# eceo-epfl/ScaleProtoSeg

Hardware: AMD Instinct MI355X
Metric: Mpix/s fwd+bwd prototype-distance, Cityscapes 1024x2048 (higher is better)
Workload: dtype bf16; 1 GPU; cityscapes_1024x2048_c256_p190_s1; latent_px_per_gpu=2097152, channels=256, prototypes=190, scales=1, classes=19, features_dtype=bf16, parallelism=single

## Files before the change

### scaleprotoseg_amd/csrc/spx_bank.hip

```cpp
#include "spx_args.h"
#include "spx_common.h"
#include <type_traits>

#define SPX_BK_THREADS 512
#define SPX_BANK_PIPE 1
#define SPX_BANK_STAGGER 1
__host__ __device__ constexpr int spx_bk_row(int cpx) { return 2 * cpx + 16; }

__host__ __device__ inline int spx_bk_wstride(const spx_plan& pl) {
    return ((pl.channels_per_scale + 31) / 32) * 32 + pl.ncb * 32 + 32;
}
static void spx_bank_parts(const spx_plan& pl, int B, int HW, int& nci, int& nci_vec, int& slabs_vec, int& slabs_tail) {
    nci = 2 * ((HW + SPX_TILE_PX - 1) / SPX_TILE_PX);
    nci_vec = HW >= 8 ? nci : 0;
    long long cap = 256 / pl.npanels;
    if (cap < 1) cap = 1;
    const long long cv = (long long)B * nci_vec, ct = (long long)B * (nci - nci_vec);
    slabs_vec = (int)(cv < cap ? cv : cap);
    slabs_tail = (int)(ct < cap ? ct : cap);
}
int spx_bank_bwd_nsplit(const spx_plan& pl, int B, int HW) {
    int nci, nci_vec, sv, st;
    spx_bank_parts(pl, B, HW, nci, nci_vec, sv, st);
    return sv + st;
}
size_t spx_bank_bwd_ws_floats(const spx_plan& pl, int nsplit) {
    return (size_t)nsplit * pl.npanels * pl.npb * 32 * spx_bk_wstride(pl);
}
template <int NPB, int NCB, bool DO_P, bool DO_W, int CPX>
__host__ __device__ constexpr int spx_bk_buf_bytes() {
    constexpr int fb = (CPX / 32) * NPB * 2 * 1024;
    return (DO_P ? fb + 256 * spx_bk_row(CPX) : 0) + (DO_W ? 2 * fb + 2 * NCB * 32 * spx_bk_row(CPX) : 0);
}
template <int NPB, int NCB, bool DO_P, bool DO_W, int CPX>
__host__ __device__ constexpr int spx_bk_lds_bytes() {
    constexpr int red = (2 * 3 * 2 * 1024 + 2 * 3 * 64) * 4;
    constexpr int n = (CPX == 32 ? 2 : 1) * spx_bk_buf_bytes<NPB, NCB, DO_P, DO_W, CPX>();
    return (n > red ? n : red) + 16;
}

template <int NPB, int NCB, bool XF32, int VM, bool DO_P, bool DO_W, bool KSPLIT, int CPX>
__global__ __launch_bounds__(SPX_BK_THREADS, 2) void spx_bank_bwd_kernel(const SpxBankBwdArgs a) {
    constexpr bool VEC = VM != 0, RAG = VM == 2;
    constexpr int SPX_BK_PX = CPX, SPX_BK_ROW = spx_bk_row(CPX);
    constexpr int NW1 = CPX / 32;
    constexpr bool PIPE = CPX == 32;
    static_assert(!(PIPE && KSPLIT), "the k-step split needs four pixel k-steps per chunk");
    extern __shared__ __attribute__((aligned(16))) char smem[];
    const spx_plan& pl = a.plan;
    const int tid = threadIdx.x, lane = tid & 63;
    const int wave = __builtin_amdgcn_readfirstlane(tid >> 6);
    const int r = lane & 31, h = lane >> 5;
    const int q = blockIdx.y, split = blockIdx.x;
    const int Cs = pl.channels_per_scale, K = pl.num_classes;
    const int C = pl.num_scales * Cs;
    const int nchb = (Cs + 31) / 32;
    constexpr int rows = NPB * 32;
    const int ch0 = pl.panel_ch0[q];
    const int tiles_per_img = (a.HW + SPX_TILE_PX - 1) / SPX_TILE_PX;
    const size_t ntiles = (size_t)a.B * tiles_per_img;
    static_assert(CPX == 64 || CPX == 32, "chunk width");
    const int nci = a.nci_launch * (64 / CPX);
    const int ci0 = a.ci_first * (64 / CPX);
    const long long total = (long long)a.B * nci;
    const long long cstep = a.nslabs;
    int phase = split;
    if (CPX == 32 && (a.nslabs & 15) == 0) {
        const int xcd = split & 7, slot = split >> 3;
        phase = 2 * ((slot >> 1) * 8 + xcd) + (slot & 1);
    }
    const long long c_begin = phase;
    const long long c_end = total;
    const bool want_w = DO_W && a.d_W != nullptr;
    const bool want_p = DO_P && a.d_bank != nullptr;
    constexpr int ESZ = XF32 ? 4 : 2;
    constexpr int NFRAG = NW1 * NPB * 2;
    constexpr int FBYTES = NFRAG * 1024;

    constexpr int BUF = spx_bk_buf_bytes<NPB, NCB, DO_P, DO_W, CPX>();
    int32_t* const ebuf = (int32_t*)(smem + spx_bk_lds_bytes<NPB, NCB, DO_P, DO_W, CPX>() - 16);
    char *Gs, *Xs, *As, *As2, *Ls, *Ls2;
    int cur_buf = 0;
    auto use_buffer = [&](int buf) {
        cur_buf = buf;
        Gs = smem + buf * BUF;
        Xs = Gs + (DO_P ? FBYTES : 0);
        As = Xs + (DO_P ? 256 * SPX_BK_ROW : 0);
        As2 = As + FBYTES;
        Ls = As2 + FBYTES;
        Ls2 = Ls + NCB * 32 * SPX_BK_ROW;
    };
    use_buffer(0);

    const int cpair = wave & 3;
    constexpr int PH = NPB / 2;
    const int pb0 = (wave >> 2) * PH;
    const bool w_role = wave < NPB;
    constexpr bool ksplit = KSPLIT;
    const int cs_first = wave >> 2;
    auto cs_owner = [&](int i) { return i == 0 ? cs_first : i + 1; };

    f32x16 accp[PH][2];
    f32x16 accw[NCB];
    float csum[PH];
    int e_acc = 0;
    bool have_e = false;
#pragma unroll
    for (int i = 0; i < PH; ++i) {
        csum[i] = 0.0f;
#pragma unroll
        for (int t = 0; t < 2; ++t)
#pragma unroll
            for (int e = 0; e < 16; ++e) accp[i][t][e] = 0.0f;
    }
#pragma unroll
    for (int cb = 0; cb < NCB; ++cb)
#pragma unroll
        for (int e = 0; e < 16; ++e) accw[cb][e] = 0.0f;

    constexpr int FP = (FBYTES / 16 + SPX_BK_THREADS - 1) / SPX_BK_THREADS;
    constexpr int PPR = CPX / 8;
    constexpr int RPP = SPX_BK_THREADS / PPR;
    constexpr int XPT = 256 / RPP;
    struct Stage {
        u32x4 gr[FP], ar[FP], xr[XPT][XF32 ? 2 : 1];
        uint32_t exw[FP];
        float lr_[(CPX * 32 * NCB + SPX_BK_THREADS - 1) / SPX_BK_THREADS];
        int32_t gexp;
        uint32_t rot_bits;
        bool ragged;
    };
    Stage stg[PIPE ? 2 : 1];
    uint32_t gsc_off[FP];
#pragma unroll
    for (int i = 0; i < FP; ++i) {
        const int off = (i * SPX_BK_THREADS + tid) * 16;
        const int frag = off >> 10, slot = (off >> 4) & 63, s2 = frag & 1;
        const int t = (slot - 8 * s2) & 63;
        const int rr = (t >> 3) * 4 + (t & 3), hh = (t & 7) >> 2;
        gsc_off[i] = off < FBYTES ? (uint32_t)(((frag >> 1) * 64 + rr + 32 * hh) * 4) : SPX_OOB;
    }
    const size_t blob_total = (size_t)pl.npanels * ntiles * 4 * NPB * 2 * 1024;
    constexpr int LPT = (SPX_BK_PX * 32 * NCB + SPX_BK_THREADS - 1) / SPX_BK_THREADS;
    const int piece = tid % PPR, prow = tid / PPR;

    long long nx_c = c_begin;
    int nx_b = (int)(c_begin / nci);
    int nx_ci = (int)(c_begin - (long long)nx_b * nci);
    const int step_b = (int)(cstep / nci), step_ci = (int)(cstep - (long long)step_b * nci);
    auto issue = [&](Stage& st) {
        const int b = nx_b;
        const int ci = ci0 + nx_ci;
        if (nx_c + cstep < c_end) {
            nx_c += cstep;
            nx_b += step_b;
            nx_ci += step_ci;
            if (nx_ci >= nci) {
                nx_ci -= nci;
                ++nx_b;
            }
        }
        constexpr int CPT = SPX_TILE_PX / CPX;
        const size_t tile_g = (size_t)b * tiles_per_img + ci / CPT;
        const size_t blob0 = ((((size_t)q * ntiles + tile_g) * 4 + NW1 * (ci % CPT)) * NPB * 2) * 1024;
        const spx_rsrc grs = make_rsrc_pred(a.g_in ? (const char*)a.g_in + blob0 : nullptr);
        const spx_rsrc ars = make_rsrc_pred(a.a_in ? (const char*)a.a_in + blob0 : nullptr);
        const char* const exsrc = (want_w && a.a_in) ? (const char*)a.a_in : nullptr;
        const spx_rsrc exs = make_rsrc_pred(exsrc ? exsrc + blob_total + blob0 / 8 : nullptr);
        st.gexp = (want_p && a.g_in) ? *(const int32_t*)((const char*)a.g_in + spx_gexp_offset(blob_total) + ((size_t)q * ntiles + tile_g) * 4) : 0;
#pragma unroll
        for (int i = 0; i < FP; ++i) {
            const uint32_t off = (uint32_t)((i * SPX_BK_THREADS + tid) * 16);
            st.gr[i] = buf_load_b128(grs, (want_p && off < (uint32_t)FBYTES) ? off : SPX_OOB, 0);
            st.exw[i] = (uint32_t)__builtin_amdgcn_raw_buffer_load_b32(exs, exsrc ? gsc_off[i] : SPX_OOB, 0, 0);
            st.ar[i] = buf_load_b128(ars, (want_w && off < (uint32_t)FBYTES) ? off : SPX_OOB, 0);
        }
        const int px = ci * SPX_BK_PX + piece * 8;
        {
            const int over = px + 8 - a.HW;
            st.rot_bits = (RAG && over > 0 && over < 8) ? (uint32_t)over * (ESZ * 8) : 0u;
            st.ragged = RAG && (ci * SPX_BK_PX + SPX_BK_PX > a.HW);
        }
#pragma unroll
        for (int i = 0; i < XPT; ++i) {
            const int row = prow + RPP * i;
            const spx_rsrc xb = make_rsrc_pred((const char*)a.x + ((size_t)b * C + ch0 + RPP * i) * a.HW * ESZ);
            const uint32_t vo = ((uint32_t)prow * (uint32_t)a.HW + (uint32_t)px) * ESZ;
            const bool row_ok = want_p && row < Cs;
            if (VEC) {
                const int over = px + 8 - a.HW;
                const uint32_t v = !row_ok ? SPX_OOB : (over <= 0 ? vo : ((RAG && over < 8) ? vo - (uint32_t)over * ESZ : SPX_OOB));
                st.xr[i][0] = buf_load_b128(xb, v, 0);
                if (XF32) st.xr[i][1] = buf_load_b128(xb, v == SPX_OOB ? SPX_OOB : v + 16, 0);
            } else if (XF32) {
#pragma unroll
                for (int e = 0; e < 8; ++e)
                    st.xr[i][e >> 2][e & 3] = __float_as_uint(buf_load_f32(xb, (row_ok && px + e < a.HW) ? vo + 4 * e : SPX_OOB, 0));
            } else {
#pragma unroll
                for (int e = 0; e < 4; ++e) {
                    const uint32_t lo = buf_load_u16(xb, (row_ok && px + 2 * e < a.HW) ? vo + 4 * e : SPX_OOB, 0);
                    const uint32_t hi = buf_load_u16(xb, (row_ok && px + 2 * e + 1 < a.HW) ? vo + 4 * e + 2 : SPX_OOB, 0);
                    st.xr[i][0][e] = lo | (hi << 16);
                }
            }
        }
        const int px0 = ci * SPX_BK_PX;
        const spx_rsrc lb = make_rsrc_pred(a.d_logits ? a.d_logits + ((size_t)b * a.HW + px0) * K : nullptr);
#pragma unroll
        for (int i = 0; i < LPT; ++i) {
            const int e = i * SPX_BK_THREADS + tid;
            const int p = e / K;
            st.lr_[i] = buf_load_f32(lb, (want_w && e < SPX_BK_PX * K && px0 + p < a.HW) ? (uint32_t)e * 4u : SPX_OOB, 0);
        }
    };

    auto commit = [&](Stage& st) {
#pragma unroll
        for (int i = 0; i < FP; ++i) {
            const int off = (i * SPX_BK_THREADS + tid) * 16;
            if (off < FBYTES) {
                if (DO_P) *(u32x4*)(Gs + off) = st.gr[i];
                if (DO_W) {
                    u32x4 ahw, alw;
                    const float asc = __builtin_amdgcn_ldexpf(1.0f / SPX_ABLOB_I16_ONE, (int)((st.exw[i] >> 8) & 0xffu) - 128);
#pragma unroll
                    for (int j = 0; j < 4; ++j) {
                        f32x2 v;
                        v[0] = (float)(short)(st.ar[i][j] & 0xffffu);
                        v[1] = (float)((int)st.ar[i][j] >> 16);
                        uint32_t hi, lo;
                        split_bf16x2(v * asc, hi, lo);
                        ahw[j] = hi;
                        alw[j] = lo;
                    }
                    *(u32x4*)(As + off) = ahw;
                    *(u32x4*)(As2 + off) = alw;
                }
            }
        }
        if (DO_P && tid == 0) ebuf[cur_buf] = st.gexp;
        if (RAG && st.ragged) {
#pragma unroll
            for (int i = 0; i < XPT; ++i) {
                if (XF32) spx_shr256(st.xr[i][0], st.xr[i][XF32 ? 1 : 0], st.rot_bits);
                else st.xr[i][0] = spx_shr128(st.xr[i][0], st.rot_bits);
            }
        }
#pragma unroll
        for (int i = 0; i < XPT; ++i) {
            u32x4 v;
            if (XF32) {
#pragma unroll
                for (int e = 0; e < 4; ++e) {
                    f32x2 p;
                    p[0] = (float)(__bf16)__uint_as_float(st.xr[i][e >> 1][(2 * e) & 3]);
                    p[1] = (float)(__bf16)__uint_as_float(st.xr[i][e >> 1][(2 * e + 1) & 3]);
                    v[e] = pack_f16x2_rtz(p);
                }
            } else {
#pragma unroll
                for (int e = 0; e < 4; ++e) v[e] = pack_f16x2_rtz(unpack_bf16x2(st.xr[i][0][e]));
            }
            if (DO_P) *(u32x4*)(Xs + (prow + RPP * i) * SPX_BK_ROW + piece * 16) = v;
        }
#pragma unroll
        for (int i = 0; i < LPT; ++i) {
            const int e = i * SPX_BK_THREADS + tid;
            if (DO_W && e < SPX_BK_PX * K) {
                const int p = e / K, cls = e - p * K;
                __bf16 hi, lo;
                split_bf16(st.lr_[i], hi, lo);
                *(uint16_t*)(Ls + cls * SPX_BK_ROW + p * 2) = __builtin_bit_cast(uint16_t, hi);
                *(uint16_t*)(Ls2 + cls * SPX_BK_ROW + p * 2) = __builtin_bit_cast(uint16_t, lo);
            }
        }
    };

    for (int buf = 0; buf < (PIPE ? 2 : 1); ++buf) {
        use_buffer(buf);
        for (int e = tid; DO_W && e < NCB * 32 * SPX_BK_PX; e += SPX_BK_THREADS) {
            const int cls = e / SPX_BK_PX, p = e - cls * SPX_BK_PX;
            if (cls >= K) {
                *(uint16_t*)(Ls + cls * SPX_BK_ROW + p * 2) = 0;
                *(uint16_t*)(Ls2 + cls * SPX_BK_ROW + p * 2) = 0;
            }
        }
    }
    use_buffer(0);

    const int tg = lane >> 4, tli = lane & 15, tqq = tli >> 2, tpp = tli & 3;
    const int ts2 = tg & 1, tkh = tg >> 1;

    auto chunk_scale = [&]() -> bool {
        const int e_c = __builtin_amdgcn_readfirstlane(ebuf[cur_buf]);
        if (have_e && e_c == e_acc) return true;
        if (have_e && e_c - e_acc > 80) return false;
        const float ratio = have_e ? __builtin_amdgcn_ldexpf(1.0f, e_c - e_acc) : 1.0f;
#pragma unroll
        for (int i = 0; i < PH; ++i) {
            csum[i] *= ratio;
#pragma unroll
            for (int t = 0; t < 2; ++t)
#pragma unroll
                for (int e = 0; e < 16; ++e) accp[i][t][e] *= ratio;
        }
        e_acc = e_c;
        have_e = true;
        return true;
    };
    auto bank_part = [&](int ks, int cp) {
        const int koff = (ks * 16 + 8 * h) * 2;
        const int pxa = ks * 16 + 8 * tkh + tqq;
        const int wsel = pxa >> 5, ra = pxa & 31;
        const int fo0 = spx_blob_slot(ra, tpp & 1, ts2) * 16 + 8 * (tpp >> 1);
        const int fo1 = spx_blob_slot(ra + 4, tpp & 1, ts2) * 16 + 8 * (tpp >> 1);
        f16x8 xb[2];
#pragma unroll
        for (int t = 0; t < 2; ++t) xb[t] = *(const f16x8*)(Xs + ((2 * cp + t) * 32 + r) * SPX_BK_ROW + koff);
#pragma unroll
        for (int i = 0; i < PH; ++i) {
            const int fb = ((wsel * NPB + pb0 + i) * 2 + ts2) * 1024;
            const s16x4 g0 = lds_tr_read(Gs + fb + fo0);
            const s16x4 g1 = lds_tr_read(Gs + fb + fo1);
            const f16x8 gf = __builtin_bit_cast(f16x8, __builtin_shufflevector(g0, g1, 0, 1, 2, 3, 4, 5, 6, 7));
            if (ksplit || cpair == cs_owner(i)) {
                f16x2 one2;
                one2[0] = (_Float16)1.0f;
                one2[1] = (_Float16)1.0f;
                float s8 = csum[i];
#pragma unroll
                for (int e = 0; e < 4; ++e) {
                    f16x2 pr;
                    pr[0] = gf[2 * e];
                    pr[1] = gf[2 * e + 1];
                    s8 = __builtin_amdgcn_fdot2(pr, one2, s8, false);
                }
                csum[i] = s8;
            }
#pragma unroll
            for (int t = 0; t < 2; ++t) accp[i][t] = __builtin_amdgcn_mfma_f32_32x32x16_f16(gf, xb[t], accp[i][t], 0, 0, 0);
        }
    };
    auto head_part = [&](int ks) {
        const int koff = (ks * 16 + 8 * h) * 2;
        const int pxa = ks * 16 + 8 * tkh + tqq;
        const int wsel = pxa >> 5, ra = pxa & 31;
        const int fo0 = spx_blob_slot(ra, tpp & 1, ts2) * 16 + 8 * (tpp >> 1);
        const int fo1 = spx_blob_slot(ra + 4, tpp & 1, ts2) * 16 + 8 * (tpp >> 1);
        const int fb = ((wsel * NPB + wave) * 2 + ts2) * 1024;
        const bf16x4 a0 = __builtin_bit_cast(bf16x4, lds_tr_read(As + fb + fo0));
        const bf16x4 a1 = __builtin_bit_cast(bf16x4, lds_tr_read(As + fb + fo1));
        const bf16x4 b0 = __builtin_bit_cast(bf16x4, lds_tr_read(As2 + fb + fo0));
        const bf16x4 b1 = __builtin_bit_cast(bf16x4, lds_tr_read(As2 + fb + fo1));
        const bf16x8 af = __builtin_shufflevector(a0, a1, 0, 1, 2, 3, 4, 5, 6, 7);
        const bf16x8 af2 = __builtin_shufflevector(b0, b1, 0, 1, 2, 3, 4, 5, 6, 7);
#pragma unroll
        for (int cb = 0; cb < NCB; ++cb) {
            const bf16x8 lf = *(const bf16x8*)(Ls + (cb * 32 + r) * SPX_BK_ROW + koff);
            const bf16x8 lf2 = *(const bf16x8*)(Ls2 + (cb * 32 + r) * SPX_BK_ROW + koff);
            accw[cb] = mfma_bf16(af, lf, accw[cb]);
            accw[cb] = mfma_bf16(af2, lf, accw[cb]);
            accw[cb] = mfma_bf16(af, lf2, accw[cb]);
        }
    };
    auto compute = [&]() {
        const bool add_p = DO_P && chunk_scale();
        if constexpr (KSPLIT) {
            if (add_p) bank_part(cpair, 0);
            if (DO_W && w_role) {
#pragma unroll
                for (int ks = 0; ks < SPX_BK_PX / 16; ++ks) head_part(ks);
            }
        } else {
#pragma unroll
            for (int ks = 0; ks < SPX_BK_PX / 16; ++ks) {
                if (add_p) bank_part(ks, cpair);
                if (DO_W && w_role) head_part(ks);
            }
        }
    };
    if constexpr (!PIPE) {
        if (c_begin < c_end) issue(stg[0]);
        for (long long c = c_begin; c < c_end; c += cstep) {
            commit(stg[0]);
            __syncthreads();
            issue(stg[0]);
            __builtin_amdgcn_sched_barrier(0);
            compute();
            __syncthreads();
        }
    } else if (c_begin < c_end) {
        const bool late = SPX_BANK_STAGGER && wave >= 4;
        const int la = late ? 1 : 0;
        issue(stg[0]);
        commit(stg[0]);
        if (!late) {
            issue(stg[0]);
            issue(stg[1]);
        } else {
            issue(stg[1]);
            issue(stg[0]);
            use_buffer(1);
            commit(stg[1]);
            issue(stg[1]);
        }
        __syncthreads();
        for (long long c = c_begin; c < c_end; c += 2 * cstep) {
            use_buffer(0);
            compute();
            if (late) __syncthreads();
            use_buffer(1 - la);
            commit(stg[0]);
            issue(stg[0]);
            if (!late) __syncthreads();
            if (c + cstep < c_end) {
                use_buffer(1);
                compute();
                if (late) __syncthreads();
                use_buffer(la);
                commit(stg[1]);
                issue(stg[1]);
                if (!late) __syncthreads();
            }
        }
    }

    if (DO_P && ksplit && want_p) {
        float* const red = (float*)smem;
        float* const redc = red + 2 * 3 * 2 * 1024;
        const int half = wave >> 2;
#pragma unroll
        for (int i = 0; i < PH; ++i) {
            __syncthreads();
            if (cpair > 0) {
#pragma unroll
                for (int t = 0; t < 2; ++t)
#pragma unroll
                    for (int reg = 0; reg < 16; ++reg)
                        red[(((half * 3 + cpair - 1) * 2 + t) * 16 + reg) * 64 + lane] = accp[i][t][reg];
                redc[(half * 3 + cpair - 1) * 64 + lane] = csum[i];
            }
            __syncthreads();
            if (cpair == 0) {
#pragma unroll
                for (int c = 0; c < 3; ++c) {
#pragma unroll
                    for (int t = 0; t < 2; ++t)
#pragma unroll
                        for (int reg = 0; reg < 16; ++reg)
                            accp[i][t][reg] += red[(((half * 3 + c) * 2 + t) * 16 + reg) * 64 + lane];
                    csum[i] += redc[(half * 3 + c) * 64 + lane];
                }
            }
        }
    }

    const int ws = spx_bk_wstride(pl);
    float* slab = a.workspace + ((size_t)(a.slab_first + split) * pl.npanels + q) * rows * ws;
    const float sinv_acc = have_e ? __builtin_amdgcn_ldexpf(1.0f, -e_acc) : 0.0f;
    if (want_p && (!ksplit || cpair == 0)) {
#pragma unroll
        for (int i = 0; i < PH; ++i) {
            const int pb = pb0 + i;
#pragma unroll
            for (int t = 0; t < 2; ++t) {
                const int chb = ksplit ? t : 2 * cpair + t;
                if (chb < nchb) {
#pragma unroll
                    for (int reg = 0; reg < 16; ++reg)
                        slab[(size_t)(pb * 32 + acc_row(reg, h)) * ws + chb * 32 + r] = accp[i][t][reg] * sinv_acc;
                }
            }
            if (ksplit ? cpair == 0 : cpair == cs_owner(i)) {
                const float s = csum[i] + __shfl_xor(csum[i], 32);
                if (h == 0) slab[(size_t)(pb * 32 + r) * ws + nchb * 32 + NCB * 32] = s * sinv_acc;
            }
        }
    }
    if (want_w && w_role) {
#pragma unroll
        for (int cb = 0; cb < NCB; ++cb) {
#pragma unroll
            for (int reg = 0; reg < 16; ++reg)
                slab[(size_t)(wave * 32 + acc_row(reg, h)) * ws + nchb * 32 + cb * 32 + r] = accw[cb][reg];
        }
    }
}

#define SPX_BD_GSLOTS 4
#define SPX_BD_XSLOTS 3
#define SPX_BD_XUNIT (256 * 128)
template <int NPB>
__host__ __device__ constexpr int spx_bd_lds_bytes() {
    return SPX_BD_GSLOTS * NPB * 2 * 1024 + SPX_BD_XSLOTS * SPX_BD_XUNIT + (SPX_BD_GSLOTS + 1) * 1024;
}

template <int NPB>
__global__ __launch_bounds__(SPX_BK_THREADS, 2) void spx_bank_dma_kernel(const SpxBankBwdArgs a) {
    extern __shared__ __attribute__((aligned(16))) char smem[];
    const spx_plan& pl = a.plan;
    const int tid = threadIdx.x, lane = tid & 63;
    const int wave = __builtin_amdgcn_readfirstlane(tid >> 6);
    const int r = lane & 31, h = lane >> 5;
    const int q = blockIdx.y, split = blockIdx.x;
    const int Cs = pl.channels_per_scale;
    const int C = pl.num_scales * Cs;
    const int nchb = (Cs + 31) / 32;
    constexpr int rows = NPB * 32;
    constexpr int GB = NPB * 2 * 1024;
    constexpr int NGP = NPB * 2 + 1;
    constexpr int PWG = (NGP + 7) / 8;
    constexpr int PW = PWG + 2;
    char* const gring = smem;
    char* const xring = smem + SPX_BD_GSLOTS * GB;
    char* const epad = xring + SPX_BD_XSLOTS * SPX_BD_XUNIT;
    char* const trash = epad + SPX_BD_GSLOTS * 1024;
    const int ch0 = pl.panel_ch0[q];
    const int tiles_per_img = (a.HW + SPX_TILE_PX - 1) / SPX_TILE_PX;
    const size_t ntiles = (size_t)a.B * tiles_per_img;
    const int nui = a.nci_launch;
    const long long total = (long long)a.B * nui;
    const long long cstep = a.nslabs;
    const long long u_begin = split;
    const int n_units = u_begin < total ? (int)((total - u_begin + cstep - 1) / cstep) : 0;
    const int n_steps = 2 * n_units;
    const size_t blob_total = (size_t)pl.npanels * ntiles * 4 * NPB * 2 * 1024;
    const int32_t* const gexp = (const int32_t*)((const char*)a.g_in + spx_gexp_offset(blob_total)) + (size_t)q * ntiles;

    const int cpair = wave & 3;
    constexpr int PH = NPB / 2;
    const int pb0 = (wave >> 2) * PH;
    const int cs_first = wave >> 2;
    auto cs_owner = [&](int i) { return i == 0 ? cs_first : i + 1; };
    f32x16 accp[PH][2];
    float csum[PH];
    int e_acc = 0;
    bool have_e = false;
#pragma unroll
    for (int i = 0; i < PH; ++i) {
        csum[i] = 0.0f;
#pragma unroll
        for (int t = 0; t < 2; ++t)
#pragma unroll
            for (int e = 0; e < 16; ++e) accp[i][t][e] = 0.0f;
    }
    for (int o = tid * 16; o < spx_bd_lds_bytes<NPB>(); o += SPX_BK_THREADS * 16) *(u32x4*)(smem + o) = u32x4{0u, 0u, 0u, 0u};
    __syncthreads();

    auto dma = [&](const char* base, uint32_t vo, char* dst) {
        const uint64_t ba = (uint64_t)base;
        u32x4 rs;
        rs[0] = __builtin_amdgcn_readfirstlane((uint32_t)ba);
        rs[1] = __builtin_amdgcn_readfirstlane((uint32_t)(ba >> 32) & 0xffffu);
        rs[2] = 0x80000000u;
        rs[3] = 0x00020000u;
        const uint32_t la = __builtin_amdgcn_readfirstlane((uint32_t)(uintptr_t)(__attribute__((address_space(3))) char*)dst);
        uint32_t keep;
        asm volatile("s_mov_b32 %0, m0\n\ts_mov_b32 m0, %1\n\ts_nop 0\n\tbuffer_load_dwordx4 %2, %3, 0 offen lds\n\ts_mov_b32 m0, %0"
                     : "=&s"(keep) : "s"(la), "v"(vo), "s"(rs) : "memory");
    };
    struct Cursor {
        int k, b, ui;
    };
    const int step_b = (int)(cstep / nui), step_ui = (int)(cstep - (long long)step_b * nui);
    auto advance = [&](Cursor& c) {
        ++c.k;
        if (c.k < n_units) {
            c.b += step_b;
            c.ui += step_ui;
            if (c.ui >= nui) {
                c.ui -= nui;
                ++c.b;
            }
        }
    };
    Cursor cg, cx;
    cg.k = cx.k = 0;
    cg.b = cx.b = (int)(u_begin / nui);
    cg.ui = cx.ui = (int)(u_begin - (long long)cg.b * nui);
    auto issue_g = [&](int gs, int e) {
        const size_t tile_g = (size_t)cg.b * tiles_per_img + (cg.ui >> 1);
        const char* const gsrc = (const char*)a.g_in + ((((size_t)q * ntiles + tile_g) * 4 + 2 * (cg.ui & 1) + e) * NPB * 2) * 1024;
#pragma unroll
        for (int i = 0; i < PWG; ++i) {
            const int p = wave + 8 * i;
            const bool is_g = p < NPB * 2, is_e = p == NPB * 2;
            dma(is_g ? gsrc + (size_t)p * 1024 : (const char*)(gexp + tile_g),
                is_g ? (uint32_t)lane * 16u : ((is_e && lane == 0) ? 0u : SPX_OOB),
                is_g ? gring + gs * GB + p * 1024 : (is_e ? epad + gs * 1024 : trash));
        }
    };
    auto issue_x = [&](int xs, int e) {
#pragma unroll
        for (int i = 0; i < 2; ++i) {
            const int p = 16 * e + wave + 8 * i;
            const int row = 8 * p + (lane >> 3);
            const int px = cx.ui * 64 + 8 * ((lane & 7) ^ ((row >> 1) & 7));
            dma((const char*)a.x + ((size_t)cx.b * C + ch0 + 8 * p) * a.HW * 2,
                (row < Cs && px + 8 <= a.HW) ? ((uint32_t)(lane >> 3) * (uint32_t)a.HW + (uint32_t)px) * 2u : SPX_OOB,
                xring + xs * SPX_BD_XUNIT + p * 1024);
        }
    };

    const int tg = lane >> 4, tli = lane & 15, tqq = tli >> 2, tpp = tli & 3;
    const int ts2 = tg & 1, tkh = tg >> 1;
    auto compute = [&](int gs, int xs, int e) {
        const char* const Gs = gring + gs * GB;
        const char* const Xs = xring + xs * SPX_BD_XUNIT;
        const int e_c = __builtin_amdgcn_readfirstlane(*(const int32_t*)(epad + gs * 1024));
        if (have_e && e_c - e_acc > 80) return;
        if (!have_e || e_c != e_acc) {
            const float ratio = have_e ? __builtin_amdgcn_ldexpf(1.0f, e_c - e_acc) : 1.0f;
#pragma unroll
            for (int i = 0; i < PH; ++i) {
                csum[i] *= ratio;
#pragma unroll
                for (int t = 0; t < 2; ++t)
#pragma unroll
                    for (int k = 0; k < 16; ++k) accp[i][t][k] *= ratio;
            }
            e_acc = e_c;
            have_e = true;
        }
#pragma unroll
        for (int ks = 0; ks < 2; ++ks) {
            const int pxa = ks * 16 + 8 * tkh + tqq;
            const int fo0 = spx_blob_slot(pxa, tpp & 1, ts2) * 16 + 8 * (tpp >> 1);
            const int fo1 = spx_blob_slot(pxa + 4, tpp & 1, ts2) * 16 + 8 * (tpp >> 1);
            f16x8 xb[2];
#pragma unroll
            for (int t = 0; t < 2; ++t) {
                const u32x4 raw = *(const u32x4*)(Xs + ((2 * cpair + t) * 32 + r) * 128 + (((4 * e + 2 * ks + h) ^ ((r >> 1) & 7)) * 16));
                u32x4 w;
#pragma unroll
                for (int k = 0; k < 4; ++k)
                    w[k] = pack_f16x2_rtz(unpack_bf16x2(raw[k]));
                xb[t] = __builtin_bit_cast(f16x8, w);
            }
#pragma unroll
            for (int i = 0; i < PH; ++i) {
                const int fb = ((pb0 + i) * 2 + ts2) * 1024;
                const s16x4 g0 = lds_tr_read(Gs + fb + fo0);
                const s16x4 g1 = lds_tr_read(Gs + fb + fo1);
                const f16x8 gf = __builtin_bit_cast(f16x8, __builtin_shufflevector(g0, g1, 0, 1, 2, 3, 4, 5, 6, 7));
                if (cpair == cs_owner(i)) {
                    f16x2 one2;
                    one2[0] = (_Float16)1.0f;
                    one2[1] = (_Float16)1.0f;
                    float s8 = csum[i];
#pragma unroll
                    for (int k = 0; k < 4; ++k) {
                        f16x2 pr;
                        pr[0] = gf[2 * k];
                        pr[1] = gf[2 * k + 1];
                        s8 = __builtin_amdgcn_fdot2(pr, one2, s8, false);
                    }
                    csum[i] = s8;
                }
#pragma unroll
                for (int t = 0; t < 2; ++t) accp[i][t] = __builtin_amdgcn_mfma_f32_32x32x16_f16(gf, xb[t], accp[i][t], 0, 0, 0);
            }
        }
    };
    if (n_steps > 0) {
        issue_g(0, 0);
        issue_x(0, 0);
        issue_x(0, 1);
        issue_g(1, 1);
        advance(cg);
        issue_g(2, 0);
        advance(cx);
        issue_x(1, 0);
        issue_x(1, 1);
        advance(cx);
        int gs = 0, xs = 0;
        for (int s = 0; s < n_steps; ++s) {
            const int e = s & 1;
            asm volatile("s_waitcnt vmcnt(%0)" ::"n"(2 * PW) : "memory");
            __builtin_amdgcn_s_waitcnt(0xc07f);
            __builtin_amdgcn_s_barrier();
            issue_g((gs + 3) & 3, 1 - e);
            if (e == 0) advance(cg);
            issue_x(xs >= 1 ? xs - 1 : 2, e);
            if (e == 1) advance(cx);
            compute(gs, xs, e);
            gs = (gs + 1) & 3;
            if (e == 1) xs = xs == 2 ? 0 : xs + 1;
        }
        asm volatile("s_waitcnt vmcnt(0)" ::: "memory");
    }

    if (!a.d_bank) return;
    const int ws = spx_bk_wstride(pl);
    float* slab = a.workspace + ((size_t)(a.slab_first + split) * pl.npanels + q) * rows * ws;
    const float sinv_acc = have_e ? __builtin_amdgcn_ldexpf(1.0f, -e_acc) : 0.0f;
#pragma unroll
    for (int i = 0; i < PH; ++i) {
        const int pb = pb0 + i;
#pragma unroll
        for (int t = 0; t < 2; ++t) {
            const int chb = 2 * cpair + t;
            if (chb < nchb) {
#pragma unroll
                for (int reg = 0; reg < 16; ++reg)
                    slab[(size_t)(pb * 32 + acc_row(reg, h)) * ws + chb * 32 + r] = accp[i][t][reg] * sinv_acc;
            }
        }
        if (cpair == cs_owner(i)) {
            const float s = csum[i] + __shfl_xor(csum[i], 32);
            if (h == 0) slab[(size_t)(pb * 32 + r) * ws + nchb * 32 + pl.ncb * 32] = s * sinv_acc;
        }
    }
}

#define SPX_RED_ELEMS 64
#define SPX_RED_PARTS 4
#define SPX_RED_FLY 8
__global__ __launch_bounds__(SPX_RED_ELEMS * SPX_RED_PARTS) void spx_bank_reduce_kernel(const SpxBankBwdArgs a) {
    __shared__ float red_s[SPX_RED_PARTS][SPX_RED_ELEMS], red_c[SPX_RED_PARTS][SPX_RED_ELEMS];
    const spx_plan& pl = a.plan;
    const int Cs = pl.channels_per_scale, K = pl.num_classes, P = pl.num_prototypes;
    const int nchb = (Cs + 31) / 32;
    const int rows = pl.npb * 32;
    const int ws = spx_bk_wstride(pl);
    const int ncols = Cs + K;
    const long long n = (long long)pl.npanels * rows * ncols;
    const int el = threadIdx.x % SPX_RED_ELEMS, part = threadIdx.x / SPX_RED_ELEMS;
    const long long gid = (long long)blockIdx.x * SPX_RED_ELEMS + el;
    const bool in = gid < n;
    const int col = in ? (int)(gid % ncols) : 0;
    const int row = in ? (int)((gid / ncols) % rows) : 0;
    const int q = in ? (int)(gid / ((long long)ncols * rows)) : 0;
    const bool is_p = col < Cs;
    const bool live = in && row < pl.panel_np[q] && (is_p ? a.d_bank != nullptr : a.d_W != nullptr);
    const size_t slab_stride = (size_t)pl.npanels * rows * ws;
    const float* base = a.workspace + ((size_t)q * rows + row) * ws;
    const int c0 = is_p ? col : nchb * 32 + (col - Cs);
    const int c1 = nchb * 32 + pl.ncb * 32;
    const int per = (a.nsplit + SPX_RED_PARTS - 1) / SPX_RED_PARTS;
    const int j0 = part * per, j1 = min(a.nsplit, j0 + per);
    float s[SPX_RED_FLY], cs[SPX_RED_FLY];
#pragma unroll
    for (int u = 0; u < SPX_RED_FLY; ++u) s[u] = cs[u] = 0.0f;
    if (live) {
        int j = j0;
        for (; j + SPX_RED_FLY <= j1; j += SPX_RED_FLY) {
            float v[SPX_RED_FLY], w[SPX_RED_FLY];
#pragma unroll
            for (int u = 0; u < SPX_RED_FLY; ++u) {
                v[u] = base[(size_t)(j + u) * slab_stride + c0];
                w[u] = base[(size_t)(j + u) * slab_stride + c1];
            }
#pragma unroll
            for (int u = 0; u < SPX_RED_FLY; ++u) {
                s[u] += v[u];
                cs[u] += w[u];
            }
        }
        for (; j < j1; ++j) {
            s[(j - j0) % SPX_RED_FLY] += base[(size_t)j * slab_stride + c0];
            cs[(j - j0) % SPX_RED_FLY] += base[(size_t)j * slab_stride + c1];
        }
    }
    red_s[part][el] = ((s[0] + s[1]) + (s[2] + s[3])) + ((s[4] + s[5]) + (s[6] + s[7]));
    red_c[part][el] = ((cs[0] + cs[1]) + (cs[2] + cs[3])) + ((cs[4] + cs[5]) + (cs[6] + cs[7]));
    __syncthreads();
    if (part != 0 || !live) return;
    float st = 0.0f, ct = 0.0f;
#pragma unroll
    for (int i = 0; i < SPX_RED_PARTS; ++i) {
        st += red_s[i][el];
        ct += red_c[i][el];
    }
    const int p = pl.panel_p0[q] + row;
    if (is_p) {
        a.d_bank[(size_t)p * Cs + col] = 2.0f * (a.bank[(size_t)p * Cs + col] * ct - st);
    } else {
        const size_t ntl = (size_t)a.B * ((a.HW + SPX_TILE_PX - 1) / SPX_TILE_PX);
        const size_t off = pl.ncb == 1 ? spx_dw_partial_bytes(pl.npanels, ntl, pl.npb, K) : spx_ablob_scale_offset(ntl * pl.npanels * 4 * pl.npb * 2 * 1024);
        a.d_W[(size_t)(col - Cs) * P + p] = *(const float*)((const char*)a.a_in + off) * st;
    }
}

__global__ __launch_bounds__(256) void spx_dw_reduce_kernel(const SpxBankBwdArgs a) {
    const spx_plan& pl = a.plan;
    const int j = blockIdx.x, q = blockIdx.y;
    const int K = pl.num_classes, NPB = pl.npb;
    const int nchb = (pl.channels_per_scale + 31) / 32;
    const int rows = NPB * 32, ws = spx_bk_wstride(pl);
    const long long ntiles = (long long)a.B * ((a.HW + SPX_TILE_PX - 1) / SPX_TILE_PX);
    const int nvb = (pl.panel_np[q] + 31) >> 5;
    const int nvec = nvb * K * 8;
    const size_t tstride = (size_t)NPB * K * 32;
    const float* const base = (const float*)a.a_in + (size_t)q * ntiles * tstride;
    float* const slab = a.workspace + ((size_t)j * pl.npanels + q) * rows * ws;
    for (int v = threadIdx.x; v < nvec; v += 256) {
        f32x4 s[8];
#pragma unroll
        for (int u = 0; u < 8; ++u) s[u] = f32x4{0.f, 0.f, 0.f, 0.f};
        long long t = j;
        for (; t + 7ll * a.nsplit < ntiles; t += 8ll * a.nsplit) {
#pragma unroll
            for (int u = 0; u < 8; ++u) s[u] += *(const f32x4*)(base + (size_t)(t + (long long)u * a.nsplit) * tstride + (size_t)v * 4);
        }
        for (int u = 0; t < ntiles; t += a.nsplit, ++u) s[u] += *(const f32x4*)(base + (size_t)t * tstride + (size_t)v * 4);
        const f32x4 tot = ((s[0] + s[1]) + (s[2] + s[3])) + ((s[4] + s[5]) + (s[6] + s[7]));
        const int pb = v / (K * 8), rem = v - pb * (K * 8), cls = rem >> 3, p4 = rem & 7;
#pragma unroll
        for (int e = 0; e < 4; ++e) slab[(size_t)(pb * 32 + p4 * 4 + e) * ws + nchb * 32 + cls] = tot[e];
    }
}

template <int NPB, int NCB, bool DO_P, bool DO_W, bool KSPLIT>
static hipError_t launch_bank_k(const SpxBankBwdArgs& a, int x_dtype, dim3 grid, hipStream_t s) {
    constexpr int CPX = (SPX_BANK_PIPE && !KSPLIT && NPB == 6 && NCB == 1 && 2 * spx_bk_buf_bytes<NPB, NCB, DO_P, DO_W, 32>() <= SPX_LDS_LIMIT) ? 32 : 64;
    constexpr size_t lds = (size_t)spx_bk_lds_bytes<NPB, NCB, DO_P, DO_W, CPX>();
    static_assert(lds <= SPX_LDS_LIMIT, "bank kernel LDS");
    spx_dispatch_x(x_dtype, a.vec_ok, [&](auto xf32, auto vm) {
        hipLaunchKernelGGL((spx_bank_bwd_kernel<NPB, NCB, decltype(xf32)::value, decltype(vm)::value, DO_P, DO_W, KSPLIT, CPX>), grid, dim3(SPX_BK_THREADS), lds, s, a);
    });
    return hipGetLastError();
}
template <int NPB, int NCB, bool DO_P, bool DO_W>
static hipError_t launch_bank_pw(const SpxBankBwdArgs& a, int x_dtype, dim3 grid, hipStream_t s) {
    if (DO_P && a.plan.channels_per_scale <= 64) return launch_bank_k<NPB, NCB, DO_P, DO_W, true>(a, x_dtype, grid, s);
    return launch_bank_k<NPB, NCB, DO_P, DO_W, false>(a, x_dtype, grid, s);
}
template <int NPB, int NCB>
static hipError_t launch_bank_x(const SpxBankBwdArgs& a, int x_dtype, dim3 grid, hipStream_t s) {
    if constexpr (NCB == 1) {
        if (!a.d_bank) return hipSuccess;
        if (x_dtype == 0 && a.vec_ok == 1 && a.HW % 64 == 0 && a.plan.channels_per_scale > 64) {
            constexpr size_t lds = (size_t)spx_bd_lds_bytes<NPB>();
            static_assert(lds <= SPX_LDS_LIMIT, "bank kernel LDS");
            hipLaunchKernelGGL((spx_bank_dma_kernel<NPB>), grid, dim3(SPX_BK_THREADS), lds, s, a);
            return hipGetLastError();
        }
        return launch_bank_pw<NPB, NCB, true, false>(a, x_dtype, grid, s);
    } else if constexpr (NCB < 5) {
        if (!a.d_bank) return launch_bank_pw<NPB, NCB, false, true>(a, x_dtype, grid, s);
        return launch_bank_pw<NPB, NCB, true, true>(a, x_dtype, grid, s);
    } else {
        hipError_t e = hipSuccess;
        if (a.d_bank) e = launch_bank_pw<NPB, NCB, true, false>(a, x_dtype, grid, s);
        if (e == hipSuccess && a.d_W) e = launch_bank_pw<NPB, NCB, false, true>(a, x_dtype, grid, s);
        return e;
    }
}

static hipError_t spx_launch_bank_part(const SpxBankBwdArgs& a, int x_dtype, hipStream_t s) {
    const spx_plan& pl = a.plan;
    dim3 grid((unsigned)a.nslabs, (unsigned)pl.npanels);
    if (pl.ncb == 1)
        return pl.npb == 2 ? launch_bank_x<2, 1>(a, x_dtype, grid, s) : pl.npb == 4 ? launch_bank_x<4, 1>(a, x_dtype, grid, s) : launch_bank_x<6, 1>(a, x_dtype, grid, s);
    if (pl.ncb == 2)
        return pl.npb == 2 ? launch_bank_x<2, 2>(a, x_dtype, grid, s) : pl.npb == 4 ? launch_bank_x<4, 2>(a, x_dtype, grid, s) : launch_bank_x<6, 2>(a, x_dtype, grid, s);
    return pl.npb == 2 ? launch_bank_x<2, 5>(a, x_dtype, grid, s) : pl.npb == 4 ? launch_bank_x<4, 5>(a, x_dtype, grid, s) : launch_bank_x<6, 5>(a, x_dtype, grid, s);
}

hipError_t spx_launch_bank_bwd(const SpxBankBwdArgs& a0, int x_dtype, hipStream_t s) {
    SpxBankBwdArgs a = a0;
    const spx_plan& pl = a.plan;
    const int rows = pl.npb * 32;
    int nci, nci_vec, sv, st;
    spx_bank_parts(pl, a.B, a.HW, nci, nci_vec, sv, st);
    a.nsplit = sv + st;
    hipError_t e = hipSuccess;
    if (sv > 0) {
        a.vec_ok = a.HW % 8 == 0 ? 1 : 2; a.ci_first = 0; a.nci_launch = nci_vec; a.slab_first = 0; a.nslabs = sv;
        e = spx_launch_bank_part(a, x_dtype, s);
    }
    if (e == hipSuccess && st > 0) {
        a.vec_ok = 0; a.ci_first = nci_vec; a.nci_launch = nci - nci_vec; a.slab_first = sv; a.nslabs = st;
        e = spx_launch_bank_part(a, x_dtype, s);
    }
    if (e != hipSuccess) return e;
    if (pl.ncb == 1 && a.d_W) {
        hipLaunchKernelGGL(spx_dw_reduce_kernel, dim3((unsigned)a.nsplit, (unsigned)pl.npanels), dim3(256), 0, s, a);
        if ((e = hipGetLastError()) != hipSuccess) return e;
    }
    const long long n = (long long)pl.npanels * rows * (pl.channels_per_scale + pl.num_classes);
    hipLaunchKernelGGL(spx_bank_reduce_kernel, dim3((unsigned)((n + SPX_RED_ELEMS - 1) / SPX_RED_ELEMS)),
                       dim3(SPX_RED_ELEMS * SPX_RED_PARTS), 0, s, a);
    return hipGetLastError();
}
```

Baseline: 826.1 Mpix/s.

## Restructure bank reduce per row with vector loads; optionally overlap dW reduce on side stream

The bank reduce kernel now assigns one block per prototype row, loading four channels per lane as a vector and reducing class columns in separate passes. This replaces the old one-element-per-thread indexing and should give more coalesced slab reads with fewer blocks. A side-stream fork is also added so the dW partial reduce can overlap with the bank partial kernels. That path is gated by SPX_SERIAL_FINISH, defaults to serial, and is skipped during graph capture.

```diff
diff --git a/scaleprotoseg_amd/csrc/spx_bank.hip b/scaleprotoseg_amd/csrc/spx_bank.hip
--- a/scaleprotoseg_amd/csrc/spx_bank.hip
+++ b/scaleprotoseg_amd/csrc/spx_bank.hip
@@ -1,5 +1,7 @@
 #include "spx_args.h"
 #include "spx_common.h"
+#include <cstdlib>
+#include <mutex>
 #include <type_traits>
 
 #define SPX_BK_THREADS 512
@@ -714,72 +716,123 @@
     }
 }
 
-#define SPX_RED_ELEMS 64
 #define SPX_RED_PARTS 4
 #define SPX_RED_FLY 8
-__global__ __launch_bounds__(SPX_RED_ELEMS * SPX_RED_PARTS) void spx_bank_reduce_kernel(const SpxBankBwdArgs a) {
-    __shared__ float red_s[SPX_RED_PARTS][SPX_RED_ELEMS], red_c[SPX_RED_PARTS][SPX_RED_ELEMS];
+#define SPX_RED_TAIL 192
+template <bool MAIN>
+__device__ __forceinline__ void spx_red_range(const float* rowp, size_t slab_stride, int j0, int j1, bool act_m, bool act_x,
+                                              int cx, int lane, f32x4& sum_m, float& sum_x) {
+    f32x4 s[SPX_RED_FLY];
+    float x[SPX_RED_FLY];
+#pragma unroll
+    for (int u = 0; u < SPX_RED_FLY; ++u) {
+        s[u] = f32x4{0.f, 0.f, 0.f, 0.f};
+        x[u] = 0.0f;
+    }
+    auto ld_m = [&](int j) { return act_m ? *(const f32x4*)(rowp + (size_t)j * slab_stride + 4 * lane) : f32x4{0.f, 0.f, 0.f, 0.f}; };
+    auto ld_x = [&](int j) { return act_x ? rowp[(size_t)j * slab_stride + cx] : 0.0f; };
+    int j = j0;
+    for (; j + 2 * SPX_RED_FLY <= j1; j += 2 * SPX_RED_FLY) {
+        f32x4 v[2 * SPX_RED_FLY];
+        float w[2 * SPX_RED_FLY];
+#pragma unroll
+        for (int u = 0; u < 2 * SPX_RED_FLY; ++u) {
+            if constexpr (MAIN) v[u] = ld_m(j + u);
+            w[u] = ld_x(j + u);
+        }
+#pragma unroll
+        for (int h = 0; h < 2; ++h) {
+#pragma unroll
+            for (int u = 0; u < SPX_RED_FLY; ++u) {
+                if constexpr (MAIN) s[u] += v[h * SPX_RED_FLY + u];
+                x[u] += w[h * SPX_RED_FLY + u];
+            }
+        }
+    }
+#pragma unroll
+    for (int h = 0; h < 2; ++h) {
+        f32x4 v[SPX_RED_FLY];
+        float w[SPX_RED_FLY];
+#pragma unroll
+        for (int u = 0; u < SPX_RED_FLY; ++u) {
+            const bool in = j + h * SPX_RED_FLY + u < j1;
+            if constexpr (MAIN) v[u] = in ? ld_m(j + h * SPX_RED_FLY + u) : f32x4{0.f, 0.f, 0.f, 0.f};
+            w[u] = in ? ld_x(j + h * SPX_RED_FLY + u) : 0.0f;
+        }
+#pragma unroll
+        for (int u = 0; u < SPX_RED_FLY; ++u) {
+            if (j + h * SPX_RED_FLY + u < j1) {
+                if constexpr (MAIN) s[u] += v[u];
+                x[u] += w[u];
+            }
+        }
+    }
+    sum_m = ((s[0] + s[1]) + (s[2] + s[3])) + ((s[4] + s[5]) + (s[6] + s[7]));
+    sum_x = ((x[0] + x[1]) + (x[2] + x[3])) + ((x[4] + x[5]) + (x[6] + x[7]));
+}
+
+__global__ __launch_bounds__(64 * SPX_RED_PARTS) void spx_bank_reduce_kernel(const SpxBankBwdArgs a) {
+    __shared__ f32x4 red_m[SPX_RED_PARTS][64];
+    __shared__ float red_x[SPX_RED_PARTS][SPX_RED_TAIL];
     const spx_plan& pl = a.plan;
     const int Cs = pl.channels_per_scale, K = pl.num_classes, P = pl.num_prototypes;
     const int nchb = (Cs + 31) / 32;
     const int rows = pl.npb * 32;
     const int ws = spx_bk_wstride(pl);
-    const int ncols = Cs + K;
-    const long long n = (long long)pl.npanels * rows * ncols;
-    const int el = threadIdx.x % SPX_RED_ELEMS, part = threadIdx.x / SPX_RED_ELEMS;
-    const long long gid = (long long)blockIdx.x * SPX_RED_ELEMS + el;
-    const bool in = gid < n;
-    const int col = in ? (int)(gid % ncols) : 0;
-    const int row = in ? (int)((gid / ncols) % rows) : 0;
-    const int q = in ? (int)(gid / ((long long)ncols * rows)) : 0;
-    const bool is_p = col < Cs;
-    const bool live = in && row < pl.panel_np[q] && (is_p ? a.d_bank != nullptr : a.d_W != nullptr);
+    const int q = blockIdx.x / rows, row = blockIdx.x % rows;
+    if (row >= pl.panel_np[q]) return;
+    const int lane = threadIdx.x & 63, part = __builtin_amdgcn_readfirstlane(threadIdx.x >> 6);
     const size_t slab_stride = (size_t)pl.npanels * rows * ws;
-    const float* base = a.workspace + ((size_t)q * rows + row) * ws;
-    const int c0 = is_p ? col : nchb * 32 + (col - Cs);
-    const int c1 = nchb * 32 + pl.ncb * 32;
+    const float* rowp = a.workspace + ((size_t)q * rows + row) * ws;
     const int per = (a.nsplit + SPX_RED_PARTS - 1) / SPX_RED_PARTS;
     const int j0 = part * per, j1 = min(a.nsplit, j0 + per);
-    float s[SPX_RED_FLY], cs[SPX_RED_FLY];
-#pragma unroll
-    for (int u = 0; u < SPX_RED_FLY; ++u) s[u] = cs[u] = 0.0f;
-    if (live) {
-        int j = j0;
-        for (; j + SPX_RED_FLY <= j1; j += SPX_RED_FLY) {
-            float v[SPX_RED_FLY], w[SPX_RED_FLY];
-#pragma unroll
-            for (int u = 0; u < SPX_RED_FLY; ++u) {
-                v[u] = base[(size_t)(j + u) * slab_stride + c0];
-                w[u] = base[(size_t)(j + u) * slab_stride + c1];
-            }
-#pragma unroll
-            for (int u = 0; u < SPX_RED_FLY; ++u) {
-                s[u] += v[u];
-                cs[u] += w[u];
-            }
-        }
-        for (; j < j1; ++j) {
-            s[(j - j0) % SPX_RED_FLY] += base[(size_t)j * slab_stride + c0];
-            cs[(j - j0) % SPX_RED_FLY] += base[(size_t)j * slab_stride + c1];
-        }
-    }
-    red_s[part][el] = ((s[0] + s[1]) + (s[2] + s[3])) + ((s[4] + s[5]) + (s[6] + s[7]));
-    red_c[part][el] = ((cs[0] + cs[1]) + (cs[2] + cs[3])) + ((cs[4] + cs[5]) + (cs[6] + cs[7]));
+    const bool want_p = a.d_bank != nullptr, want_w = a.d_W != nullptr;
+    const bool act_m = want_p && 4 * lane < nchb * 32;
+    const int tcs = pl.ncb * 32;
+    const int pass_m = want_p ? tcs >> 6 : -1;
+    const int npass = max(want_w ? (K + 63) >> 6 : 0, pass_m + 1);
+    for (int g = 0; g < npass; ++g) {
+        const int t = g * 64 + lane;
+        const bool act_x = (want_w && t < K) || (want_p && t == tcs);
+        f32x4 sm;
+        float sx;
+        if (g == pass_m) {
+            spx_red_range<true>(rowp, slab_stride, j0, j1, act_m, act_x, nchb * 32 + t, lane, sm, sx);
+            red_m[part][lane] = sm;
+        } else {
+            spx_red_range<false>(rowp, slab_stride, j0, j1, false, act_x, nchb * 32 + t, lane, sm, sx);
+        }
+        red_x[part][t] = sx;
+    }
     __syncthreads();
-    if (part != 0 || !live) return;
-    float st = 0.0f, ct = 0.0f;
-#pragma unroll
-    for (int i = 0; i < SPX_RED_PARTS; ++i) {
-        st += red_s[i][el];
-        ct += red_c[i][el];
-    }
     const int p = pl.panel_p0[q] + row;
-    if (is_p) {
-        a.d_bank[(size_t)p * Cs + col] = 2.0f * (a.bank[(size_t)p * Cs + col] * ct - st);
+    if (part == 0) {
+        if (!act_m) return;
+        f32x4 st = f32x4{0.f, 0.f, 0.f, 0.f};
+        float ct = 0.0f;
+#pragma unroll
+        for (int i = 0; i < SPX_RED_PARTS; ++i) {
+            st += red_m[i][lane];
+            ct += red_x[i][tcs];
+        }
+        const float* bk = a.bank + (size_t)p * Cs;
+        float* out = a.d_bank + (size_t)p * Cs;
+        if ((Cs & 3) == 0) {
+            if (4 * lane < Cs) *(f32x4*)(out + 4 * lane) = 2.0f * (*(const f32x4*)(bk + 4 * lane) * ct - st);
+        } else {
+#pragma unroll
+            for (int e = 0; e < 4; ++e)
+                if (4 * lane + e < Cs) out[4 * lane + e] = 2.0f * (bk[4 * lane + e] * ct - st[e]);
+        }
     } else {
+        const int c = (int)threadIdx.x - 64;
+        if (!want_w || c >= K) return;
+        float st = 0.0f;
+#pragma unroll
+        for (int i = 0; i < SPX_RED_PARTS; ++i) st += red_x[i][c];
         const size_t ntl = (size_t)a.B * ((a.HW + SPX_TILE_PX - 1) / SPX_TILE_PX);
         const size_t off = pl.ncb == 1 ? spx_dw_partial_bytes(pl.npanels, ntl, pl.npb, K) : spx_ablob_scale_offset(ntl * pl.npanels * 4 * pl.npb * 2 * 1024);
-        a.d_W[(size_t)(col - Cs) * P + p] = *(const float*)((const char*)a.a_in + off) * st;
+        a.d_W[(size_t)c * P + p] = *(const float*)((const char*)a.a_in + off) * st;
     }
 }
 
@@ -859,6 +912,57 @@
     return pl.npb == 2 ? launch_bank_x<2, 5>(a, x_dtype, grid, s) : pl.npb == 4 ? launch_bank_x<4, 5>(a, x_dtype, grid, s) : launch_bank_x<6, 5>(a, x_dtype, grid, s);
 }
 
+#define SPX_MAX_DEVICES 64
+static std::mutex g_side_mu;
+static struct { hipStream_t stream; bool tried; } g_side[SPX_MAX_DEVICES];
+
+static bool spx_serial_finish() {
+    static const bool serial = [] {
+        const char* e = getenv("SPX_SERIAL_FINISH");
+        return !(e && e[0] == '0' && e[1] == 0);
+    }();
+    return serial;
+}
+static hipStream_t spx_side_stream() {
+    int dev = -1;
+    if (hipGetDevice(&dev) != hipSuccess || dev < 0 || dev >= SPX_MAX_DEVICES) return nullptr;
+    std::lock_guard<std::mutex> lock(g_side_mu);
+    if (!g_side[dev].tried) {
+        g_side[dev].tried = true;
+        if (hipStreamCreateWithFlags(&g_side[dev].stream, hipStreamNonBlocking) != hipSuccess) g_side[dev].stream = nullptr;
+    }
+    return g_side[dev].stream;
+}
+static hipError_t spx_launch_dw_reduce(const SpxBankBwdArgs& a, hipStream_t s) {
+    hipLaunchKernelGGL(spx_dw_reduce_kernel, dim3((unsigned)a.nsplit, (unsigned)a.plan.npanels), dim3(256), 0, s, a);
+    return hipGetLastError();
+}
+static bool spx_dw_fork(const SpxBankBwdArgs& a, hipStream_t s, hipStream_t* side, hipEvent_t* join) {
+    hipStreamCaptureStatus cap = hipStreamCaptureStatusActive;
+    hipEvent_t fork = nullptr;
+    *join = nullptr;
+    const bool ok = hipStreamIsCapturing(s, &cap) == hipSuccess && cap == hipStreamCaptureStatusNone &&
+                    (*side = spx_side_stream()) != nullptr &&
+                    hipEventCreateWithFlags(&fork, hipEventDisableTiming) == hipSuccess &&
+                    hipEventCreateWithFlags(join, hipEventDisableTiming) == hipSuccess &&
+                    hipEventRecord(fork, s) == hipSuccess && hipStreamWaitEvent(*side, fork, 0) == hipSuccess &&
+                    spx_launch_dw_reduce(a, *side) == hipSuccess;
+    if (fork) (void)hipEventDestroy(fork);
+    if (!ok) {
+        if (*join) (void)hipEventDestroy(*join);
+        *join = nullptr;
+        (void)hipGetLastError();
+    }
+    return ok;
+}
+static hipError_t spx_dw_join(hipStream_t s, hipStream_t side, hipEvent_t join) {
+    const bool ok = hipEventRecord(join, side) == hipSuccess && hipStreamWaitEvent(s, join, 0) == hipSuccess;
+    (void)hipEventDestroy(join);
+    if (ok) return hipSuccess;
+    (void)hipGetLastError();
+    return hipStreamSynchronize(side);
+}
+
 hipError_t spx_launch_bank_bwd(const SpxBankBwdArgs& a0, int x_dtype, hipStream_t s) {
     SpxBankBwdArgs a = a0;
     const spx_plan& pl = a.plan;
@@ -866,6 +970,10 @@
     int nci, nci_vec, sv, st;
     spx_bank_parts(pl, a.B, a.HW, nci, nci_vec, sv, st);
     a.nsplit = sv + st;
+    const bool dw_sum = pl.ncb == 1 && a.d_W;
+    hipStream_t side = nullptr;
+    hipEvent_t join = nullptr;
+    const bool forked = dw_sum && a.d_bank && !spx_serial_finish() && spx_dw_fork(a, s, &side, &join);
     hipError_t e = hipSuccess;
     if (sv > 0) {
         a.vec_ok = a.HW % 8 == 0 ? 1 : 2; a.ci_first = 0; a.nci_launch = nci_vec; a.slab_first = 0; a.nslabs = sv;
@@ -875,13 +983,12 @@
         a.vec_ok = 0; a.ci_first = nci_vec; a.nci_launch = nci - nci_vec; a.slab_first = sv; a.nslabs = st;
         e = spx_launch_bank_part(a, x_dtype, s);
     }
+    if (forked) {
+        const hipError_t ej = spx_dw_join(s, side, join);
+        if (e == hipSuccess) e = ej;
+    }
     if (e != hipSuccess) return e;
-    if (pl.ncb == 1 && a.d_W) {
-        hipLaunchKernelGGL(spx_dw_reduce_kernel, dim3((unsigned)a.nsplit, (unsigned)pl.npanels), dim3(256), 0, s, a);
-        if ((e = hipGetLastError()) != hipSuccess) return e;
-    }
-    const long long n = (long long)pl.npanels * rows * (pl.channels_per_scale + pl.num_classes);
-    hipLaunchKernelGGL(spx_bank_reduce_kernel, dim3((unsigned)((n + SPX_RED_ELEMS - 1) / SPX_RED_ELEMS)),
-                       dim3(SPX_RED_ELEMS * SPX_RED_PARTS), 0, s, a);
+    if (dw_sum && !forked && (e = spx_launch_dw_reduce(a, s)) != hipSuccess) return e;
+    hipLaunchKernelGGL(spx_bank_reduce_kernel, dim3((unsigned)(pl.npanels * rows)), dim3(64 * SPX_RED_PARTS), 0, s, a);
     return hipGetLastError();
 }
```

Result: no change. 827.5 Mpix/s, median of 6 (+0.2%).
